# filippo-orru/path-tracer-rust

Hardware: AMD Instinct MI355X
Metric: ray_bounces_per_sec (higher is better)
Workload: dtype f32

## Files before the change

### path-tracer-rust_amd/csrc/pt_api.hip

```cpp
#include <cerrno>
#include <chrono>
#include <cstdio>
#include <cstdlib>
#include <cstring>
#include <map>
#include <string>
#include <thread>
#include <vector>

#include "../../include/ptrace.h"
#include "pt_accum.h"
#include "pt_aov.h"
#include "pt_denoise.h"
#include "pt_host.h"
#include "pt_kernels.h"
#include "pt_masked.h"
#include "pt_noise.h"
#include "pt_present.h"
#include "pt_probe.h"
#include "pt_refit.h"
#include "pt_reproject.h"
#include "pt_upsample.h"
#include "pt_tile.h"

// ... 1366 lines not shown
        HIP_TRY(hipMemcpy(c->d_sph.p, fs.sph_pairs.data(), fs.sph_pairs.size() * sizeof(SphPairRec), hipMemcpyHostToDevice));
    if (!fs.flat_pairs.empty())
        HIP_TRY(hipMemcpy(c->d_flat.p, fs.flat_pairs.data(), fs.flat_pairs.size() * sizeof(FlatPairRec), hipMemcpyHostToDevice));
    if (!fs.cand_pairs.empty())
        HIP_TRY(hipMemcpy(c->d_cand.p, fs.cand_pairs.data(), fs.cand_pairs.size() * sizeof(CandPairRec), hipMemcpyHostToDevice));
    HIP_TRY(hipMemcpy(c->d_rank_id.p, fs.rank_id.data(), fs.rank_id.size() * sizeof(uint32_t), hipMemcpyHostToDevice));
    c->scene.sph_pairs = c->d_sph.p;
    c->scene.flat_pairs = c->d_flat.p;
    c->scene.cand_pairs = c->d_cand.p;
    HIP_TRY(hipMemcpy(c->d_surf.p, fs.surf.data(), fs.surf.size() * sizeof(SurfRec), hipMemcpyHostToDevice));
    HIP_TRY(hipMemcpy(c->d_tri_rank.p, fs.tri_rank.data(), fs.tri_rank.size() * sizeof(uint32_t), hipMemcpyHostToDevice));
    c->scene.rank_id = c->d_rank_id.p;
    c->scene.tri_rank = c->d_tri_rank.p;
    if (!fs.bvh_meshes.empty())
        HIP_TRY(hipMemcpy(c->d_bvh_meshes.p, fs.bvh_meshes.data(), fs.bvh_meshes.size() * sizeof(BvhMeshRec), hipMemcpyHostToDevice));
    c->scene.bvh_meshes = c->d_bvh_meshes.p;
    c->scene.n_bvh_meshes = (uint32_t)fs.bvh_meshes.size();
    c->scene.surf = c->d_surf.p;
    c->scene.n_sph_pairs = (uint32_t)fs.sph_pairs.size();
    c->scene.n_flat_pairs = (uint32_t)fs.flat_pairs.size();
    c->scene.n_cand_pairs = (uint32_t)fs.cand_pairs.size();
    c->scene.n_other_pairs = fs.n_other_pairs;
    c->scene.n_flat_exact = fs.n_flat_exact;
    c->scene.nodes_in_lds_ok = c->tune.nodes_lds ? 1u : 0u;
    set_glass_defer(c, objs, n_objs);
    c->cand_ok = fs.cand_ok;
    c->scene.cand_staged = 0u;
    c->scene.surf_staged = 0u;
    c->scene.surf_head = 0u;
    c->scene.walk_queue_cap = c->tune.walk_queue_cap;
#ifdef PT_WALK_STATS
    if (!c->scene.stats) {
        HIP_TRY(hipMalloc((void **)&c->scene.stats, 16 * sizeof(unsigned long long)));
        HIP_TRY(hipMemset(c->scene.stats, 0, 16 * sizeof(unsigned long long)));
    }
#endif
#ifdef PT_PHASE_STATS
    if (!c->scene.phase_stats) {
        HIP_TRY(hipMalloc((void **)&c->scene.phase_stats, (kPhCount * 3 + 2) * sizeof(unsigned long long)));
        HIP_TRY(hipMemset(c->scene.phase_stats, 0, (kPhCount * 3 + 2) * sizeof(unsigned long long)));
    }
#endif
    c->n_bvh_nodes = (uint32_t)fs.bvh_nodes.size();
    c->scene.bvh_nodes = c->d_nodes.p;
    c->scene.n_bvh_nodes = c->n_bvh_nodes;
    c->scene.planar = 1u;
// ... 144 lines not shown
    if (moved) {
        HIP_TRY(hipMemcpy(c->d_opairs.p + e.obj_pair, &fs.obj_pairs[e.obj_pair], sizeof(ObjPairRec), hipMemcpyHostToDevice));
        if (e.on_device) {
            HIP_TRY(hipMemcpy(c->d_bvh_meshes.p + e.bvh_mesh, &fs.bvh_meshes[e.bvh_mesh], sizeof(BvhMeshRec), hipMemcpyHostToDevice));
        } else {
            int rc;
            if ((rc = c->d_sph.ensure(fs.sph_pairs.size())) || (rc = c->d_flat.ensure(fs.flat_pairs.size())) ||
                (rc = c->d_cand.ensure(fs.cand_pairs.size())))
                return rc;
            if (!fs.sph_pairs.empty())
                HIP_TRY(hipMemcpy(c->d_sph.p, fs.sph_pairs.data(), fs.sph_pairs.size() * sizeof(SphPairRec), hipMemcpyHostToDevice));
            if (!fs.flat_pairs.empty())
                HIP_TRY(hipMemcpy(c->d_flat.p, fs.flat_pairs.data(), fs.flat_pairs.size() * sizeof(FlatPairRec), hipMemcpyHostToDevice));
            if (!fs.cand_pairs.empty())
                HIP_TRY(hipMemcpy(c->d_cand.p, fs.cand_pairs.data(), fs.cand_pairs.size() * sizeof(CandPairRec), hipMemcpyHostToDevice));
            c->scene.sph_pairs = c->d_sph.p;
            c->scene.flat_pairs = c->d_flat.p;
            c->scene.cand_pairs = c->d_cand.p;
            c->scene.n_sph_pairs = (uint32_t)fs.sph_pairs.size();
            c->scene.n_flat_pairs = (uint32_t)fs.flat_pairs.size();
            c->scene.n_cand_pairs = (uint32_t)fs.cand_pairs.size();
            c->scene.n_other_pairs = fs.n_other_pairs;
            c->scene.n_flat_exact = fs.n_flat_exact;
            c->cand_ok = fs.cand_ok;
            c->scene.cand_scan = cand_scan_for(c, 0u);
            c->table_count[PT_TABLE_SPH_PAIRS] = fs.sph_pairs.size();
            c->table_count[PT_TABLE_FLAT_PAIRS] = fs.flat_pairs.size();
            c->table_count[PT_TABLE_CAND_PAIRS] = fs.cand_pairs.size();
            if (o.kind == PT_MESH && o.tri_count != 0u) {
                const ObjRec &r = fs.objs[index];
                HIP_TRY(hipMemcpy(c->d_tris.p + r.pair_begin, &fs.tri_pairs[r.pair_begin], (size_t)r.pair_count * sizeof(TriPairRec),
                                  hipMemcpyHostToDevice));
                HIP_TRY(hipMemcpy(c->d_tshade.p + o.tri_offset, &fs.tri_shade[o.tri_offset], (size_t)o.tri_count * sizeof(TriShade),
                                  hipMemcpyHostToDevice));
            }
        }
    }
    if (!e.surf.empty())
        HIP_TRY(hipMemcpy(c->d_surf.p + e.rank, e.surf.data(), e.surf.size() * sizeof(SurfRec), hipMemcpyHostToDevice));
    if (!e.tail.empty())
        HIP_TRY(hipMemcpy(c->d_surf.p + e.tail_at, e.tail.data(), e.tail.size() * sizeof(SurfRec), hipMemcpyHostToDevice));
    if (e.on_device) {
        if (moved) {
            pt_ctx::DevRefit *d = nullptr;
            const int rc = refit_plan_for(c, index, &d);
            if (rc) return rc;
// ... 1495 lines not shown
```

### path-tracer-rust_amd/csrc/pt_device.h

```cpp
#pragma once

#include "pt_math.h"

namespace pt {

constexpr uint32_t kKindSphere = 0u, kKindMesh = 1u;
constexpr uint32_t kDiffuse = 0u, kSpecular = 1u, kRefract = 2u;
constexpr int kMaxDepth = 12;

struct alignas(16) ObjRec {
    float cx, cy, cz;
    float rr;
    uint32_t kind;
    uint32_t tri_begin;
    uint32_t tri_count;
    uint32_t pair_begin;
    uint32_t pair_count;
    int32_t bvh_root;
    float rr_in;
    uint32_t pad1;
};

struct alignas(16) ObjPairRec {
    float cx[2], cy[2], cz[2];
    float rr[2];
// ... 106 lines not shown
    const TriShade *tri_shade;
    const BvhNode *bvh_nodes;
    const BvhNode4 *bvh_nodes4;
    uint32_t n_bvh_nodes4;
    uint32_t n_objs;
    uint32_t n_tris;
    uint32_t n_bvh_nodes;
    uint32_t bvh_in_lds;
    uint32_t bvh_pair_base;
    uint32_t bvh_stack;
    uint32_t leaf_quorum;
    uint32_t planar;
    const SphPairRec *sph_pairs;
    const FlatPairRec *flat_pairs;
    const CandPairRec *cand_pairs;
    const uint32_t *rank_id;
    const SurfRec *surf;
    const uint32_t *tri_rank;
    const BvhMeshRec *bvh_meshes;
    uint32_t n_bvh_meshes;
    uint32_t n_sph_pairs, n_flat_pairs, n_cand_pairs;
    uint32_t n_other_pairs;
    uint32_t n_flat_exact;
    uint32_t glass_defer_ok;
    uint32_t nodes_in_lds_ok;
    uint32_t cand_scan;
    uint32_t cand_staged;
    uint32_t surf_staged;
    uint32_t surf_head;
    uint32_t walk_queue_cap;
#ifdef PT_WALK_STATS
    unsigned long long *stats;
#endif
#ifdef PT_PHASE_STATS
    unsigned long long *phase_stats;
#endif
};
#ifdef PT_PHASE_STATS
enum : uint32_t {
    kPhOther = 0, kPhLoad, kPhSpheres, kPhFilter, kPhBatch, kPhFinish, kPhSurface, kPhRng, kPhDiffuse, kPhSpecular, kPhGlass,
    kPhAppend, kPhDefer, kPhBarrier, kPhWants, kPhWalkGate, kPhWalkBox, kPhWalkLeaf, kPhPrimary, kPhEmit,
    kPhPush, kPhAppend2, kPhRoulette, kPhEmitAdd, kPhCount
};
struct PhaseLds {
    unsigned long long state[4];
    unsigned long long cyc[4][kPhCount];
// ... 161 lines not shown
__device__ __forceinline__ void phase_end(unsigned long long *out, unsigned long long t0, unsigned long long r0) {
    phase_to(kPhOther);
    PhaseLds &P = phase_lds();
    const uint32_t w = threadIdx.x >> 6, lane = threadIdx.x & 63u;
    for (uint32_t k = lane; k < kPhCount; k += 64u) {
        const unsigned long long c = *(volatile unsigned long long *)&P.cyc[w][k], n = *(volatile unsigned long long *)&P.cnt[w][k];
        if (c) atomicAdd(out + 3u * k, c);
        if (n) {
            atomicAdd(out + 3u * k + 1u, n >> 32);
            atomicAdd(out + 3u * k + 2u, n & 0xffffffffull);
        }
    }
    if (lane == 0u) {
        atomicAdd(out + kPhCount * 3u, (unsigned long long)(__builtin_amdgcn_s_memtime() - t0));
        atomicAdd(out + kPhCount * 3u + 1u, (unsigned long long)(__builtin_amdgcn_s_memrealtime() - r0));
    }
}
#endif

typedef float f32x2 __attribute__((ext_vector_type(2)));
__device__ __forceinline__ f32x2 splat2(float v) {
    f32x2 r = {v, v};
    return r;
}
template <class T>
__device__ __forceinline__ T ld_uniform(const T *p) {
    static_assert(sizeof(T) % 16 == 0 && alignof(T) >= 16, "records are whole 16-byte rows");
    typedef uint32_t row_t __attribute__((ext_vector_type(4)));
    union {
        T v;
        row_t w[sizeof(T) / 16];
    } u;
    const __attribute__((address_space(4))) row_t *q =
        (const __attribute__((address_space(4))) row_t *)(unsigned long long)p;
#pragma unroll
    for (uint32_t i = 0; i < sizeof(T) / 16; ++i) u.w[i] = q[i];
    return u.v;
}
__device__ __forceinline__ f32x2 ld2(const float (&p)[2]) {
    f32x2 r = {p[0], p[1]};
    return r;
}
__device__ __forceinline__ f32x2 f_rcp2(f32x2 d) {
    const f32x2 one = splat2(1.0f);
    const f32x2 r0 = {__builtin_amdgcn_rcpf(d[0]), __builtin_amdgcn_rcpf(d[1])};
    const f32x2 e0 = __builtin_elementwise_fma(-d, r0, one);
// ... 818 lines not shown
            const float sq = f_sqrt(det);
            suspect = !(!(det < 0.0f) && ((b - sq) >= 1e-4f || (b + sq) >= 1e-4f));
        }
    }
    if (__builtin_amdgcn_ballot_w64(suspect) != 0ull) h = scan_scene<BVH, true, DEFER_WALK>(S, o, d, lds, want_walk);
    return h;
}

struct CandLds {
    unsigned long long *keys;
    float4 *ray_a;
    float2 *ray_b;
    uint16_t *queue;
    const CandPairRec *staged;
    const SurfRec *surf;
};
constexpr unsigned long long kKeyMiss = 0x7f800000ffffffffull;

struct CandRing {
    uint32_t head, count;
};

template <int AXIS, bool EXACT>
__device__ __forceinline__ void filter_flat(const FlatPairRec &f, vec3 o, vec3 d, vec3 inv, float bound, uint64_t valid_m,
                                            uint64_t graze, uint64_t *m0, uint64_t *m1) {
    const float oa = AXIS == 0 ? o.x : (AXIS == 1 ? o.y : o.z), ob = AXIS == 0 ? o.y : (AXIS == 1 ? o.z : o.x),
                oc = AXIS == 0 ? o.z : (AXIS == 1 ? o.x : o.y);
    const float db = AXIS == 0 ? d.y : (AXIS == 1 ? d.z : d.x), dc = AXIS == 0 ? d.z : (AXIS == 1 ? d.x : d.y);
    const float ia = AXIS == 0 ? inv.x : (AXIS == 1 ? inv.y : inv.z);
    const f32x2 tv = ld2(f.pc) - splat2(oa);
    const f32x2 t2 = tv * splat2(ia);
    const f32x2 yb = __builtin_elementwise_fma(splat2(db), t2, splat2(ob)) - ld2(f.cb);
    const f32x2 zc = __builtin_elementwise_fma(splat2(dc), t2, splat2(oc)) - ld2(f.cc);
    const f32x2 lim = splat2(bound) + ld2(f.tpad);
    uint64_t in[2];
    if (EXACT) {
#pragma unroll
        for (int hf = 0; hf < 2; ++hf)
            in[hf] = __builtin_amdgcn_ballot_w64(f_abs(yb[hf]) <= f.hb[hf]) & __builtin_amdgcn_ballot_w64(f_abs(zc[hf]) <= f.hc[hf]) &
                     __builtin_amdgcn_ballot_w64(t2[hf] <= lim[hf]);
        const uint64_t fwd0 = __builtin_amdgcn_ballot_w64(t2[0] > 0.0f), fwd1 = __builtin_amdgcn_ballot_w64(t2[1] > 0.0f);
        *m0 = f.pair[0] != kNoPair ? ((graze | in[0]) & fwd0 & valid_m) : 0ull;
        *m1 = f.pair[1] != kNoPair ? ((graze | in[1]) & fwd1 & valid_m) : 0ull;
        return;
    }
#pragma unroll
    for (int hf = 0; hf < 2; ++hf)
        in[hf] = __builtin_amdgcn_ballot_w64(f_abs(yb[hf]) <= f.hb[hf]) & __builtin_amdgcn_ballot_w64(f_abs(zc[hf]) <= f.hc[hf]) &
                 __builtin_amdgcn_ballot_w64(t2[hf] >= -f.tpad[hf]) & __builtin_amdgcn_ballot_w64(t2[hf] <= lim[hf]);
    *m0 = f.pair[0] != kNoPair ? ((graze | in[0]) & valid_m) : 0ull;
    *m1 = f.pair[1] != kNoPair ? ((graze | in[1]) & valid_m) : 0ull;
}

__device__ __forceinline__ unsigned long long cand_spheres(const DevScene &S, vec3 o, vec3 d, float *best_out) {
    float best_t = __builtin_inff();
    uint32_t best_rank = 0xffffffffu;
    const f32x2 ox2 = splat2(o.x), oy2 = splat2(o.y), oz2 = splat2(o.z);
    const f32x2 dx2 = splat2(d.x), dy2 = splat2(d.y), dz2 = splat2(d.z);
    for (uint32_t p = 0; p < S.n_sph_pairs; ++p) {
        const SphPairRec sp = ld_uniform(S.sph_pairs + p);
        const f32x2 opx = ld2(sp.cx) - ox2, opy = ld2(sp.cy) - oy2, opz = ld2(sp.cz) - oz2;
        const f32x2 b = (opx * dx2 + opy * dy2) + opz * dz2;
        const f32x2 det = (b * b - ((opx * opx + opy * opy) + opz * opz)) + ld2(sp.rr);
#pragma unroll
        for (int hf = 0; hf < 2; ++hf) {
            if (__builtin_amdgcn_ballot_w64(!(det[hf] < 0.0f)) == 0ull) continue;
            const float sq = f_sqrt(det[hf]);
            const float t0 = b[hf] - sq, t1 = b[hf] + sq;
            const bool near_ok = t0 >= 1e-4f, far_ok = t1 >= 1e-4f;
            const float t = near_ok ? t0 : t1;
            if (far_ok && t < best_t) {
                best_t = t;
                best_rank = sp.rank[hf];
            }
        }
    }
    *best_out = best_t;
    return ((unsigned long long)__float_as_uint(best_t) << 32) | best_rank;
}

template <bool STAGED>
__device__ __forceinline__ void cand_batch(const DevScene &S, const CandLds &L, CandRing &R, uint32_t lane, uint32_t count) {
    PT_PHASE_N(kPhBatch, count);
    const bool valid = lane < count;
    const uint32_t at = (R.head + lane) & (kCandQueueCap - 1u);
    R.head = (R.head + count) & (kCandQueueCap - 1u);
    R.count -= count;
    if (valid) {
        const uint32_t ent = (uint32_t)L.queue[at];
        const uint32_t slot = ent & 127u, q = ent >> 7;
        const float4 ra = L.ray_a[slot];
        const float2 rb = L.ray_b[slot];
        const vec3 ro = mk(ra.x, ra.y, ra.z), rd = mk(ra.w, rb.x, rb.y);
        CandPairRec tr;
        if (STAGED)
            tr = L.staged[q];
        else
            tr = S.cand_pairs[q];
        unsigned long long keys2[2];
        float t_hit[2];
        pair_test_keys(tr, ro, rd, keys2, t_hit);
        const bool first = keys2[0] <= keys2[1];
        const unsigned long long kmin = first ? keys2[0] : keys2[1];
        const float mt = first ? t_hit[0] : t_hit[1];
        bool pass = (uint32_t)(kmin >> 32) < 0x7f800000u;
        const vec3 g = mk(tr.gx, tr.gy, tr.gz);
        const vec3 pc = (ro + rd * mt) - g;
        const bool deep = dot(pc, pc) <= tr.grr_in;
        if (pass && !deep) {
            const vec3 og = g - ro;
            const float b = dot(og, rd);
            const float det = (b * b - dot(og, og)) + tr.grr;
            const float sq = f_sqrt(det);
            pass = !(det < 0.0f) && ((b - sq) >= 1e-4f || (b + sq) >= 1e-4f);
        }
        if (pass) atomicMin(&L.keys[slot], kmin + (1ull << 32));
    }
}

template <bool STAGED>
__device__ __forceinline__ void cand_filter_and_drain(const DevScene &S, const CandLds &L, CandRing &R, uint32_t lane,
                                                      uint32_t par, bool valid, vec3 o, vec3 d, float bound) {
    auto push2 = [&](uint64_t m0, uint32_t q0, uint64_t m1, uint32_t q1) {
        if ((m0 | m1) == 0ull) return;
        const uint32_t n0 = (uint32_t)__builtin_popcountll(m0);
        const uint32_t base = R.head + R.count;
        const uint32_t me = lane | (par << 6);
        if (__builtin_amdgcn_inverse_ballot_w64(m0)) {
            PT_PHASE(kPhPush);
            const uint32_t at = (base + __builtin_amdgcn_mbcnt_hi((uint32_t)(m0 >> 32), __builtin_amdgcn_mbcnt_lo((uint32_t)m0, 0u))) & (kCandQueueCap - 1u);
            L.queue[at] = (uint16_t)(me | (q0 << 7));
        }
        if (__builtin_amdgcn_inverse_ballot_w64(m1)) {
            PT_PHASE(kPhPush);
            const uint32_t at = (base + n0 + __builtin_amdgcn_mbcnt_hi((uint32_t)(m1 >> 32), __builtin_amdgcn_mbcnt_lo((uint32_t)m1, 0u))) & (kCandQueueCap - 1u);
            L.queue[at] = (uint16_t)(me | (q1 << 7));
        }
        PT_PHASE(kPhFilter);
        R.count += n0 + (uint32_t)__builtin_popcountll(m1);
    };
    auto drain = [&]() {
#ifdef PT_PHASE_STATS
        const bool any = R.count >= 64u;
#endif
        while (R.count >= 64u) cand_batch<STAGED>(S, L, R, lane, 64u);
#ifdef PT_PHASE_STATS
        if (any) PT_PHASE(kPhFilter);
#endif
    };
    PT_PHASE(kPhFilter);
    const vec3 inv = mk(__builtin_amdgcn_rcpf(d.x), __builtin_amdgcn_rcpf(d.y), __builtin_amdgcn_rcpf(d.z));
    const uint64_t valid_m = __builtin_amdgcn_ballot_w64(valid);
    const uint64_t gz_x = __builtin_amdgcn_ballot_w64(!(f_abs(d.x) >= kGrazing)), gz_y = __builtin_amdgcn_ballot_w64(!(f_abs(d.y) >= kGrazing)),
                   gz_z = __builtin_amdgcn_ballot_w64(!(f_abs(d.z) >= kGrazing));
    for (uint32_t p = 0; p < S.n_flat_exact; ++p) {
        const FlatPairRec f = ld_uniform(S.flat_pairs + p);
        uint64_t m0, m1;
        if (f.axis == 0u)
            filter_flat<0, true>(f, o, d, inv, bound, valid_m, gz_x, &m0, &m1);
        else if (f.axis == 1u)
            filter_flat<1, true>(f, o, d, inv, bound, valid_m, gz_y, &m0, &m1);
        else
            filter_flat<2, true>(f, o, d, inv, bound, valid_m, gz_z, &m0, &m1);
        push2(m0, f.pair[0], m1, f.pair[1]);
        drain();
    }
    for (uint32_t p = S.n_flat_exact; p < S.n_flat_pairs; ++p) {
        const FlatPairRec f = ld_uniform(S.flat_pairs + p);
        uint64_t m0, m1;
        if (f.axis == 0u)
            filter_flat<0, false>(f, o, d, inv, bound, valid_m, gz_x, &m0, &m1);
        else if (f.axis == 1u)
            filter_flat<1, false>(f, o, d, inv, bound, valid_m, gz_y, &m0, &m1);
        else
            filter_flat<2, false>(f, o, d, inv, bound, valid_m, gz_z, &m0, &m1);
        push2(m0, f.pair[0], m1, f.pair[1]);
        drain();
    }
    for (uint32_t q = 0; q < S.n_other_pairs; ++q) {
        push2(valid_m, q, 0ull, 0u);
        drain();
    }
}

__device__ __forceinline__ bool walk_deferred(const DevScene &S, vec3 o, vec3 d, uint4 *lds, float &best_t,
                                              int32_t &best_id, const LeafLds *leaves = nullptr) {
    bool tie = false;
    const uint32_t n_pairs = (S.n_objs + 1u) >> 1;
    for (uint32_t p = 0; p < n_pairs; ++p) {
        const ObjPairRec ob = ld_uniform(S.obj_pairs + p);
#pragma unroll
        for (int hf = 0; hf < 2; ++hf) {
            const int32_t root = ob.bvh_root[hf];
            if (ob.kind[hf] != kKindMesh || root == kNoBvh) continue;
            const vec3 op = mk(ob.cx[hf], ob.cy[hf], ob.cz[hf]) - o;
            const float b = dot(op, d);
            const float det = (b * b - dot(op, op)) + ob.rr[hf];
            const float sq = f_sqrt(det);
            const bool pass = !(det < 0.0f) && ((b - sq) >= 1e-4f || (b + sq) >= 1e-4f);
            if (__builtin_amdgcn_ballot_w64(pass) == 0ull) continue;
            float mt = __builtin_inff();
            int32_t mid = -1;
            if (pass) {
                bvh_walk(S, lds, o, d, root, best_t, mt, mid, leaves);
            }
// ... 317 lines not shown
```

### path-tracer-rust_amd/csrc/pt_host.cpp

```cpp
#include "pt_host.h"
#include "pt_denoise.h"
#include "pt_masked.h"
#include "pt_present.h"
#include "pt_probe.h"
#include "pt_refit.h"
#include "pt_reproject.h"
#include "pt_upsample.h"

#include <algorithm>
#include <cmath>
#include <cstring>
#include <limits>

namespace pt {
namespace host {

static vec3 ld(const float *p) { return mk(p[0], p[1], p[2]); }
static void st(float *p, vec3 v) {
    p[0] = v.x;
    p[1] = v.y;
    p[2] = v.z;
}

void camera_basis(const pt_camera &cam, float lens_center[3], float su_out[3], float sv_out[3]) {
// ... 486 lines not shown
                const uint32_t hf = fill[a] & 1u;
                f.pc[hf] = lov[a];
                f.cb[hf] = 0.5f * (lov[b] + hiv[b]);
                f.hb[hf] = 0.5f * (hiv[b] - lov[b]) + pad + 4.0f * e * (f_abs(lov[b]) + f_abs(hiv[b]));
                f.cc[hf] = 0.5f * (lov[c] + hiv[c]);
                f.hc[hf] = 0.5f * (hiv[c] - lov[c]) + pad + 4.0f * e * (f_abs(lov[c]) + f_abs(hiv[c]));
                f.tpad[hf] = pad;
                for (int h2 = 0; h2 < 2; ++h2) {
                    if (tp.id[h2] == kNoTri) continue;
                    const float e1v[3] = {tp.e1x[h2], tp.e1y[h2], tp.e1z[h2]}, e2v[3] = {tp.e2x[h2], tp.e2y[h2], tp.e2z[h2]};
                    const double pa = (double)e1v[b] * e2v[c], pb = (double)e1v[c] * e2v[b];
                    if (!(std::fabs(pa - pb) >= 1e-3 * (std::fabs(pa) + std::fabs(pb))) || !std::isfinite(pa) || !std::isfinite(pb))
                        f.sign_exact = 0u;
                }
                f.pair[hf] = (uint32_t)filtered.size();
                filtered.push_back(cand_rec(i, pp));
                ++fill[a];
            }
        }
        for (int a = 0; a < 3; ++a) out.flat_pairs.insert(out.flat_pairs.end(), by_axis[a].begin(), by_axis[a].end());
        out.n_flat_exact = (uint32_t)(std::stable_partition(out.flat_pairs.begin(), out.flat_pairs.end(),
                                                            [](const FlatPairRec &f) { return f.sign_exact != 0u; }) -
                                      out.flat_pairs.begin());
        out.n_other_pairs = (uint32_t)out.cand_pairs.size();
        for (FlatPairRec &f : out.flat_pairs)
            for (int hf = 0; hf < 2; ++hf)
                if (f.pair[hf] != kNoPair) f.pair[hf] += out.n_other_pairs;
        out.cand_pairs.insert(out.cand_pairs.end(), filtered.begin(), filtered.end());
        out.cand_ok = out.cand_pairs.size() <= kCandMaxPairs;
    }
}

const char *bad_material(const pt_object &o) {
    for (float v : o.color)
        if (!finite_nonneg(v)) return "color";
    for (float v : o.emission)
        if (!finite_nonneg(v)) return "emission";
    return nullptr;
}

bool flatten_scene(const pt_camera &cam, const pt_object *objs, uint32_t n_objs, const pt_triangle *tris,
                   uint32_t n_tris, FlatScene &out, std::string &err, const Reach *origin_box, Reach *used) {
    if (n_objs >= (1u << 30) || n_tris >= (1u << 30)) {
        err = "scene too large";
        return false;
    }
// ... 1129 lines not shown
```

### path-tracer-rust_amd/csrc/pt_host.h

```cpp
#pragma once

#include <algorithm>
#include <string>
#include <vector>

#include "../../include/ptrace.h"
#include "pt_device.h"
#include "pt_refit.h"

namespace pt {

void set_error(const std::string &m);
inline int refuse(const char *why) {
    set_error(why);
    return PT_ERR_INVALID;
}

namespace host {

struct FlatScene {
    std::vector<ObjRec> objs;
    std::vector<ObjPairRec> obj_pairs;
    std::vector<TriPairRec> tri_pairs;
    std::vector<MatRec> mats;
    std::vector<TriShade> tri_shade;
    std::vector<BvhNode> bvh_nodes;
    std::vector<BvhNode4> bvh_nodes4;
    std::vector<SphPairRec> sph_pairs;
    std::vector<FlatPairRec> flat_pairs;
    std::vector<CandPairRec> cand_pairs;
    std::vector<uint32_t> rank_id;
    std::vector<SurfRec> surf;
    std::vector<uint32_t> tri_rank;
    std::vector<BvhMeshRec> bvh_meshes;
    std::vector<uint32_t> wide_src;
    uint32_t n_other_pairs = 0;
    uint32_t n_flat_exact = 0;
    bool cand_ok = false;
    uint32_t bvh_stack = 0;
    uint32_t bvh_pair_base = 0;
    uint32_t bvh_pair_span = 0;
};

void camera_basis(const pt_camera &cam, float lens_center[3], float su[3], float sv[3]);
void mesh_bounding_sphere(const pt_triangle *tris, uint32_t n, float center[3], float *radius);
void mesh_bounding_box(const pt_triangle *tris, uint32_t n, pt_triangle out[12]);
void box_pair_records(const pt_triangle box[12], const float position[3], TriPairRec out[6]);
bool bvh_refs_fit(uint64_t n_nodes, uint64_t n_pair_records);

struct PassPlanIn {
    uint64_t npix = 0;
    uint32_t spp = 0;
    uint64_t want = 0;
    bool want_is_default = true;
    bool stack_form = false;
    bool stack_park = false;
    bool cand_scan = false, has_bvh = false;
    uint64_t streams = 0;
    uint32_t per_stream = 0;
    uint32_t wave_stack = 0;
// ... 211 lines not shown
```

### path-tracer-rust_amd/csrc/pt_kernels.hip

```cpp
#include <cstdio>
#include <cstdlib>
#include <string>

#include "pt_kernels.h"
#ifdef PT_TU_TILE
#include "pt_tile.h"
#endif

namespace pt {

#ifdef PT_TU_TILE
typedef TileParams MegaParams;
#define k_mega k_tile_mega
#define k_mega_cand k_tile_mega_cand
#else
typedef FrameParams MegaParams;
#endif
#if defined(PT_TU_FLAT) || defined(PT_TU_TILE)
#define PT_TU_PART 1
#endif

void set_error(const std::string &m);

extern __shared__ uint4 dyn_lds[];
// ... 12 lines not shown
__device__ __forceinline__ StreamSlice slice_of(const RayQueue &q, uint32_t b, uint32_t cap) {
    StreamSlice s;
    s.base = q.buf + (size_t)b * cap * kRayBytes;
    s.off_tp = cap * 16u;
    s.off_od1 = cap * 32u;
    return s;
}
__device__ __forceinline__ float4 ld_od0(const StreamSlice &q, uint32_t i) { return *reinterpret_cast<const float4 *>(q.base + i * 16u); }
__device__ __forceinline__ float4 ld_tp(const StreamSlice &q, uint32_t i) { return *reinterpret_cast<const float4 *>(q.base + (i * 16u + q.off_tp)); }
__device__ __forceinline__ float2 ld_od1(const StreamSlice &q, uint32_t i) { return *reinterpret_cast<const float2 *>(q.base + (i * 8u + q.off_od1)); }
__device__ __forceinline__ void store_ray(const StreamSlice &q, uint32_t slot, vec3 o, vec3 d, vec3 thr, uint32_t word) {
    *reinterpret_cast<float4 *>(q.base + slot * 16u) = make_float4(o.x, o.y, o.z, d.x);
    *reinterpret_cast<float2 *>(q.base + (slot * 8u + q.off_od1)) = make_float2(d.y, d.z);
    *reinterpret_cast<float4 *>(q.base + (slot * 16u + q.off_tp)) = make_float4(thr.x, thr.y, thr.z, __uint_as_float(word));
}
__device__ __forceinline__ void load_ray_slice(const StreamSlice &q, uint32_t i, vec3 &o, vec3 &d, vec3 &thr, uint32_t &word) {
    const float4 a = ld_od0(q, i);
    const float4 tp = ld_tp(q, i);
    const float2 c = ld_od1(q, i);
    o = mk(a.x, a.y, a.z);
    d = mk(a.w, c.x, c.y);
    thr = mk(tp.x, tp.y, tp.z);
    word = __float_as_uint(tp.w);
}

#ifndef PT_TU_PART
template <bool PROBE>
__global__ __launch_bounds__(kBlock) void k_generate(FrameParams F, RayQueue q, uint32_t *__restrict__ cnt0,
                                                     uint32_t cap, uint32_t s0, uint32_t s_here, uint32_t m) {
    const uint32_t b = blockIdx.x, tid = threadIdx.x;
    const StreamSlice qs = slice_of(q, b, cap);
    const uint32_t mb = stream_pixel_count(F.npix, F.n_streams, b);
    const uint32_t n = mb * s_here;
    for (uint32_t g = tid; g < n; g += kBlock) {
        const uint32_t pl = stream_pixel(F.n_streams, b, g % mb);
        const uint32_t s = s0 + g / mb;
        const PathRay r = primary_ray<PROBE>(F, global_pixel(F, pl), s);
        store_ray(qs, g, r.o, r.d, r.thr, pack_word(g % mb, g / mb, PROBE ? F.depth0 : 0u, 1u));
    }
    if (tid == 0) cnt0[b] = n;
}

constexpr uint32_t kParkCap = 128;
__host__ __device__ inline size_t bvh_park_offset(const DevScene &S, uint32_t block) {
    return (bvh_lds_bytes(S, block) + 15) & ~(size_t)15;
}
// ... 657 lines not shown
        const uint32_t phi = 2u * top + 4u * (n_park + n_defer + (pending ? 64u : 0u));
        const bool may_start = gen_left != 0u && (room_for_all || phi + 256u <= room);
        uint32_t src = 0u, cnt = 0u;
        if (top >= 64u) {
            src = 1u;
            cnt = 64u;
        } else if (may_start) {
            src = 2u;
            cnt = gen_left < 64u ? gen_left : 64u;
        } else if (top != 0u) {
            src = 1u;
            cnt = top;
        }
        src = rfl(src);
        cnt = rfl(cnt);
        const bool idle = src == 0u && !pending;
        if (idle && n_defer == 0u && n_park == 0u) break;
        const bool cur_valid = lane < cnt;
        vec3 cur_thr = mk(0.0f, 0.0f, 0.0f);
        uint32_t word = 0;
        const uint32_t pend_entries = ring.count;
        bool ran_batch = false;
        if (src != 0u) {
            PathRay in;
            in.o = in.d = in.thr = mk(0.0f, 0.0f, 0.0f);
            if (src == 2u) {
                PT_PHASE(kPhPrimary);
                if (cur_valid) {
                    const uint32_t pj = gen_pj, sj = gen_sj;
                    FrameParams Fl;
                    {
                        const float4 c0 = *reinterpret_cast<const float4 *>(s_tail_p + 4), c1 = *reinterpret_cast<const float4 *>(s_tail_p + 8),
                                     c2 = *reinterpret_cast<const float4 *>(s_tail_p + 12);
                        Fl.lens_x = c0.x, Fl.lens_y = c0.y, Fl.lens_z = c0.z, Fl.cam_px = c0.w, Fl.cam_py = c1.x, Fl.cam_pz = c1.y;
                        Fl.su_x = c1.z, Fl.su_y = c1.w, Fl.su_z = c2.x, Fl.sv_x = c2.y, Fl.sv_y = c2.z, Fl.sv_z = c2.w;
                        Fl.width = s_tail_p[16], Fl.height = s_tail_p[17];
                        Fl.seed_lo = P.seed_lo, Fl.seed_hi = P.seed_hi;
                    }
                    in = PROBE ? primary_ray<PROBE>(F, lds_pix[pj], s0 + sj) : primary_ray_at(Fl, lds_pix[pj], lds_px[pj], lds_py[pj], s0 + sj);
                    word = pack_word(pj, sj, PROBE ? F.depth0 : 0u, 1u);
                }
#if PT_SAMPLE_MAJOR
                gen_sj += step_r;
                gen_pj += step_q;
                if (gen_sj >= s_here) {
                    gen_sj -= s_here;
                    gen_pj += 1u;
                }
#else
                gen_pj += step_r;
                gen_sj += step_q;
                if (gen_pj >= mb) {
                    gen_pj -= mb;
                    gen_sj += 1u;
                }
#endif
                gen_left = rfl(gen_left - cnt);
            } else {
                PT_PHASE(kPhLoad);
                __builtin_amdgcn_fence(__ATOMIC_RELEASE, "wavefront");
                __builtin_amdgcn_fence(__ATOMIC_ACQUIRE, "wavefront");
                top = rfl(top - cnt);
                if (cur_valid) load_ray_slice(qs, top + lane, in.o, in.d, in.thr, word);
            }
            total += cnt;
            cur_thr = in.thr;
            const uint32_t slot = (par << 6) | lane;
            cand.ray_a[slot] = make_float4(in.o.x, in.o.y, in.o.z, in.d.x);
            cand.ray_b[slot] = make_float2(in.d.y, in.d.z);
            float bound;
            PT_PHASE(kPhSpheres);
            const unsigned long long key0 = cand_spheres(S, in.o, in.d, &bound);
            cand.keys[slot] = cur_valid ? key0 : kKeyMiss;
            const uint32_t before = ring.head;
            cand_filter_and_drain<STAGED>(S, cand, ring, lane, par, cur_valid, in.o, in.d, bound);
            ran_batch = ring.head != before;
        }
        if (pending) {
            PT_PHASE(kPhFinish);
            if (pend_entries != 0u && !ran_batch) cand_batch<STAGED>(S, cand, ring, lane, ring.count);
            PT_PHASE(kPhFinish);
            ShadeOut so;
            so.n_rays = 0;
            so.emits = false;
            so.deferred = false;
            float hit_t = 0.0f;
            uint32_t hit_rank = 0xffffffffu;
            PathRay pr;
            pr.o = pr.d = pr.thr = mk(0.0f, 0.0f, 0.0f);
            bool park = false;
            unsigned long long park_key = 0ull;
            if (prev_valid) {
                const uint32_t slot = ((par ^ 1u) << 6) | lane;
                const unsigned long long key = load_key(&cand.keys[slot]);
                const uint32_t rank = (uint32_t)key;
                if (BVH) {
                    const float4 ra = cand.ray_a[slot];
                    const float2 rb = cand.ray_b[slot];
// ... 1146 lines not shown
```

### path-tracer-rust_amd/host/object_check.cpp

```cpp
#include "check_common.h"
#include "../csrc/pt_host.h"

using namespace pt;
using host::FlatScene;
using host::Reach;

template <class T>
static bool same_table(const std::vector<T> &a, const std::vector<T> &b) {
    return a.size() == b.size() && (a.empty() || memcmp(a.data(), b.data(), a.size() * sizeof(T)) == 0);
}

struct Scene {
    pt_camera cam;
    std::vector<pt_object> objs;
    std::vector<pt_triangle> tris;
};

static void terrain(uint32_t q, uint32_t n, uint32_t seed, std::vector<pt_triangle> &out) {
    std::vector<float> h((size_t)(q + 1u) * (q + 1u));
    uint32_t s = seed;
    for (float &v : h) v = (float)(lcg(s) >> 26) * 0.125f;
    auto vert = [&](uint32_t i, uint32_t j, float v[3]) {
        v[0] = (float)i * 0.375f - 1.0f, v[1] = h[(size_t)i * (q + 1u) + j], v[2] = (float)j * 0.625f - 2.0f;
    };
// ... 55 lines not shown
static bool flatten(const Scene &sc, FlatScene &fs, const Reach *B, Reach *used) {
    std::string err;
    return host::flatten_scene(sc.cam, sc.objs.data(), (uint32_t)sc.objs.size(), sc.tris.data(), (uint32_t)sc.tris.size(), fs, err, B, used);
}

static bool same_tables(const FlatScene &a, const FlatScene &b) {
    const struct {
        const char *name;
        bool same;
    } t[] = {{"objs", same_table(a.objs, b.objs)},
             {"obj_pairs", same_table(a.obj_pairs, b.obj_pairs)},
             {"tri_pairs", same_table(a.tri_pairs, b.tri_pairs)},
             {"mats", same_table(a.mats, b.mats)},
             {"tri_shade", same_table(a.tri_shade, b.tri_shade)},
             {"bvh_nodes", same_table(a.bvh_nodes, b.bvh_nodes)},
             {"bvh_nodes4", same_table(a.bvh_nodes4, b.bvh_nodes4)},
             {"sph_pairs", same_table(a.sph_pairs, b.sph_pairs)},
             {"flat_pairs", same_table(a.flat_pairs, b.flat_pairs)},
             {"cand_pairs", same_table(a.cand_pairs, b.cand_pairs)},
             {"rank_id", same_table(a.rank_id, b.rank_id)},
             {"surf", same_table(a.surf, b.surf)},
             {"tri_rank", same_table(a.tri_rank, b.tri_rank)},
             {"bvh_meshes", same_table(a.bvh_meshes, b.bvh_meshes)},
             {"the counts", a.n_other_pairs == b.n_other_pairs && a.n_flat_exact == b.n_flat_exact && a.cand_ok == b.cand_ok}};
    for (const auto &x : t)
        if (!x.same) {
            fprintf(stderr, "same_tables: %s differ\n", x.name);
            return false;
        }
    return true;
}

static bool same_small_tables(const FlatScene &a, const FlatScene &b) {
    return same_table(a.mats, b.mats) && same_table(a.tri_shade, b.tri_shade) && same_table(a.sph_pairs, b.sph_pairs) &&
           same_table(a.flat_pairs, b.flat_pairs) && same_table(a.cand_pairs, b.cand_pairs) && same_table(a.surf, b.surf) &&
           a.n_other_pairs == b.n_other_pairs && a.n_flat_exact == b.n_flat_exact && a.cand_ok == b.cand_ok;
}

static bool same_spheres(const FlatScene &a, const FlatScene &b) {
    if (a.objs.size() != b.objs.size() || a.bvh_meshes.size() != b.bvh_meshes.size()) return false;
    for (size_t i = 0; i < a.objs.size(); ++i) {
        const float x[5] = {a.objs[i].cx, a.objs[i].cy, a.objs[i].cz, a.objs[i].rr, a.objs[i].rr_in};
        const float y[5] = {b.objs[i].cx, b.objs[i].cy, b.objs[i].cz, b.objs[i].rr, b.objs[i].rr_in};
        const ObjPairRec &p = a.obj_pairs[(a.objs.size() - 1u - i) / 2u], &q = b.obj_pairs[(a.objs.size() - 1u - i) / 2u];
        const size_t hf = (a.objs.size() - 1u - i) & 1u;
        if (memcmp(x, y, sizeof x) != 0 || p.cx[hf] != q.cx[hf] || p.cy[hf] != q.cy[hf] || p.cz[hf] != q.cz[hf] || p.rr[hf] != q.rr[hf] ||
            p.admit[hf] != q.admit[hf] || p.obj[hf] != q.obj[hf])
            return false;
    }
    for (size_t m = 0; m < a.bvh_meshes.size(); ++m)
        if (memcmp(&a.bvh_meshes[m], &b.bvh_meshes[m], 4 * sizeof(float)) != 0) return false;
    return true;
}

static bool refit_is_sound(const FlatScene &a, const FlatScene &b, const Scene &sc, const Reach &B) {
    const float scene_R = length(mk(B.hi[0] - B.lo[0], B.hi[1] - B.lo[1], B.hi[2] - B.lo[2]));
    std::vector<const TriPairRec *> rec_b(sc.tris.size(), nullptr);
    std::vector<uint32_t> half_b(sc.tris.size(), 0u), owner(sc.tris.size(), 0u);
    for (const TriPairRec &r : b.tri_pairs)
// ... 266 lines not shown
```

Before: 56.00 billion.

## Pack ray into paired registers and split exact flat filtering per axis

Ray origin and direction are carried as three packed float pairs, with empty asm pins so the compiler keeps them as paired VGPRs for packed math in the sphere and flat-pair filter loops. The exact flat-pair loop is split into three axis-specialised runs using per-axis counts computed on the host, which removes the per-pair axis branch. The ray slice load becomes unconditional with a clamped lane index, and the valid mask comes from a lane-count compare instead of a ballot. The per-axis loops assume exact pairs are grouped by axis after the host partition. Pinning may also raise register pressure.

```diff
diff --git a/path-tracer-rust_amd/csrc/pt_api.hip b/path-tracer-rust_amd/csrc/pt_api.hip
--- a/path-tracer-rust_amd/csrc/pt_api.hip
+++ b/path-tracer-rust_amd/csrc/pt_api.hip
@@ -1412,6 +1412,7 @@
     c->scene.n_cand_pairs = (uint32_t)fs.cand_pairs.size();
     c->scene.n_other_pairs = fs.n_other_pairs;
     c->scene.n_flat_exact = fs.n_flat_exact;
+    for (int k = 0; k < 3; ++k) c->scene.n_flat_exact_axis[k] = fs.n_flat_exact_axis[k];
     c->scene.nodes_in_lds_ok = c->tune.nodes_lds ? 1u : 0u;
     set_glass_defer(c, objs, n_objs);
     c->cand_ok = fs.cand_ok;
@@ -1602,6 +1603,7 @@
             c->scene.n_cand_pairs = (uint32_t)fs.cand_pairs.size();
             c->scene.n_other_pairs = fs.n_other_pairs;
             c->scene.n_flat_exact = fs.n_flat_exact;
+            for (int k = 0; k < 3; ++k) c->scene.n_flat_exact_axis[k] = fs.n_flat_exact_axis[k];
             c->cand_ok = fs.cand_ok;
             c->scene.cand_scan = cand_scan_for(c, 0u);
             c->table_count[PT_TABLE_SPH_PAIRS] = fs.sph_pairs.size();
diff --git a/path-tracer-rust_amd/csrc/pt_device.h b/path-tracer-rust_amd/csrc/pt_device.h
--- a/path-tracer-rust_amd/csrc/pt_device.h
+++ b/path-tracer-rust_amd/csrc/pt_device.h
@@ -1,6 +1,8 @@
 #pragma once
 
 #include "pt_math.h"
+
+#include <type_traits>
 
 namespace pt {
 
@@ -153,6 +155,7 @@
     uint32_t n_sph_pairs, n_flat_pairs, n_cand_pairs;
     uint32_t n_other_pairs;
     uint32_t n_flat_exact;
+    uint32_t n_flat_exact_axis[3];
     uint32_t glass_defer_ok;
     uint32_t nodes_in_lds_ok;
     uint32_t cand_scan;
@@ -360,6 +363,49 @@
 __device__ __forceinline__ f32x2 splat2(float v) {
     f32x2 r = {v, v};
     return r;
+}
+typedef float f32x4 __attribute__((ext_vector_type(4)));
+struct RayRows {
+    f32x2 p0, p1;
+    f32x2 p2;
+};
+enum : int { kRayOx = 0, kRayOy, kRayOz, kRayDx, kRayDy, kRayDz };
+__device__ __forceinline__ RayRows ray_rows(vec3 o, vec3 d) {
+    RayRows r;
+    r.p0 = f32x2{o.x, o.y};
+    r.p1 = f32x2{o.z, d.x};
+    r.p2 = f32x2{d.y, d.z};
+    return r;
+}
+template <int C>
+__device__ __forceinline__ float ray_get(const RayRows &r) {
+    static_assert(C >= 0 && C < 6, "o.x, o.y, o.z, d.x, d.y, d.z");
+    if constexpr (C < 2)
+        return r.p0[C];
+    else if constexpr (C < 4)
+        return r.p1[C - 2];
+    else
+        return r.p2[C - 4];
+}
+__device__ __forceinline__ void pin_pair(f32x2 &p) { asm volatile("" : "+v"(p)); }
+__device__ __forceinline__ void pin_rows(RayRows &r) {
+    pin_pair(r.p0);
+    pin_pair(r.p1);
+    pin_pair(r.p2);
+}
+template <int H>
+__device__ __forceinline__ f32x2 rep2(f32x2 p) {
+    return __builtin_shufflevector(p, p, H, H);
+}
+template <int C>
+__device__ __forceinline__ f32x2 ray_rep(const RayRows &r) {
+    static_assert(C >= 0 && C < 6, "o.x, o.y, o.z, d.x, d.y, d.z");
+    if constexpr (C < 2)
+        return rep2<C>(r.p0);
+    else if constexpr (C < 4)
+        return rep2<C - 2>(r.p1);
+    else
+        return rep2<C - 4>(r.p2);
 }
 template <class T>
 __device__ __forceinline__ T ld_uniform(const T *p) {
@@ -1224,17 +1270,21 @@
 };
 
 template <int AXIS, bool EXACT>
-__device__ __forceinline__ void filter_flat(const FlatPairRec &f, vec3 o, vec3 d, vec3 inv, float bound, uint64_t valid_m,
+__device__ __forceinline__ void filter_flat(const FlatPairRec &f, const RayRows &ray, f32x2 inv_xy, f32x2 inv_zb, uint64_t valid_m,
                                             uint64_t graze, uint64_t *m0, uint64_t *m1) {
-    const float oa = AXIS == 0 ? o.x : (AXIS == 1 ? o.y : o.z), ob = AXIS == 0 ? o.y : (AXIS == 1 ? o.z : o.x),
-                oc = AXIS == 0 ? o.z : (AXIS == 1 ? o.x : o.y);
-    const float db = AXIS == 0 ? d.y : (AXIS == 1 ? d.z : d.x), dc = AXIS == 0 ? d.z : (AXIS == 1 ? d.x : d.y);
-    const float ia = AXIS == 0 ? inv.x : (AXIS == 1 ? inv.y : inv.z);
-    const f32x2 tv = ld2(f.pc) - splat2(oa);
-    const f32x2 t2 = tv * splat2(ia);
-    const f32x2 yb = __builtin_elementwise_fma(splat2(db), t2, splat2(ob)) - ld2(f.cb);
-    const f32x2 zc = __builtin_elementwise_fma(splat2(dc), t2, splat2(oc)) - ld2(f.cc);
-    const f32x2 lim = splat2(bound) + ld2(f.tpad);
+    constexpr int A = AXIS, B = (AXIS + 1) % 3, C = (AXIS + 2) % 3;
+    const f32x2 oa = ray_rep<kRayOx + A>(ray), ob = ray_rep<kRayOx + B>(ray), oc = ray_rep<kRayOx + C>(ray);
+    const f32x2 db = ray_rep<kRayDx + B>(ray), dc = ray_rep<kRayDx + C>(ray);
+    f32x2 ia;
+    if constexpr (A < 2)
+        ia = rep2<A>(inv_xy);
+    else
+        ia = rep2<0>(inv_zb);
+    const f32x2 tv = ld2(f.pc) - oa;
+    const f32x2 t2 = tv * ia;
+    const f32x2 yb = __builtin_elementwise_fma(db, t2, ob) - ld2(f.cb);
+    const f32x2 zc = __builtin_elementwise_fma(dc, t2, oc) - ld2(f.cc);
+    const f32x2 lim = rep2<1>(inv_zb) + ld2(f.tpad);
     uint64_t in[2];
     if (EXACT) {
 #pragma unroll
@@ -1254,13 +1304,14 @@
     *m1 = f.pair[1] != kNoPair ? ((graze | in[1]) & valid_m) : 0ull;
 }
 
-__device__ __forceinline__ unsigned long long cand_spheres(const DevScene &S, vec3 o, vec3 d, float *best_out) {
+__device__ __forceinline__ unsigned long long cand_spheres(const DevScene &S, RayRows &r, float *best_out) {
     float best_t = __builtin_inff();
     uint32_t best_rank = 0xffffffffu;
-    const f32x2 ox2 = splat2(o.x), oy2 = splat2(o.y), oz2 = splat2(o.z);
-    const f32x2 dx2 = splat2(d.x), dy2 = splat2(d.y), dz2 = splat2(d.z);
     for (uint32_t p = 0; p < S.n_sph_pairs; ++p) {
         const SphPairRec sp = ld_uniform(S.sph_pairs + p);
+        pin_rows(r);
+        const f32x2 ox2 = ray_rep<kRayOx>(r), oy2 = ray_rep<kRayOy>(r), oz2 = ray_rep<kRayOz>(r);
+        const f32x2 dx2 = ray_rep<kRayDx>(r), dy2 = ray_rep<kRayDy>(r), dz2 = ray_rep<kRayDz>(r);
         const f32x2 opx = ld2(sp.cx) - ox2, opy = ld2(sp.cy) - oy2, opz = ld2(sp.cz) - oz2;
         const f32x2 b = (opx * dx2 + opy * dy2) + opz * dz2;
         const f32x2 det = (b * b - ((opx * opx + opy * opy) + opz * opz)) + ld2(sp.rr);
@@ -1279,6 +1330,10 @@
     }
     *best_out = best_t;
     return ((unsigned long long)__float_as_uint(best_t) << 32) | best_rank;
+}
+__device__ __forceinline__ unsigned long long cand_spheres(const DevScene &S, vec3 o, vec3 d, float *best_out) {
+    RayRows r = ray_rows(o, d);
+    return cand_spheres(S, r, best_out);
 }
 
 template <bool STAGED>
@@ -1322,7 +1377,7 @@
 
 template <bool STAGED>
 __device__ __forceinline__ void cand_filter_and_drain(const DevScene &S, const CandLds &L, CandRing &R, uint32_t lane,
-                                                      uint32_t par, bool valid, vec3 o, vec3 d, float bound) {
+                                                      uint32_t par, uint64_t valid_m, const RayRows &ray, float bound) {
     auto push2 = [&](uint64_t m0, uint32_t q0, uint64_t m1, uint32_t q1) {
         if ((m0 | m1) == 0ull) return;
         const uint32_t n0 = (uint32_t)__builtin_popcountll(m0);
@@ -1351,31 +1406,36 @@
 #endif
     };
     PT_PHASE(kPhFilter);
-    const vec3 inv = mk(__builtin_amdgcn_rcpf(d.x), __builtin_amdgcn_rcpf(d.y), __builtin_amdgcn_rcpf(d.z));
-    const uint64_t valid_m = __builtin_amdgcn_ballot_w64(valid);
-    const uint64_t gz_x = __builtin_amdgcn_ballot_w64(!(f_abs(d.x) >= kGrazing)), gz_y = __builtin_amdgcn_ballot_w64(!(f_abs(d.y) >= kGrazing)),
-                   gz_z = __builtin_amdgcn_ballot_w64(!(f_abs(d.z) >= kGrazing));
-    for (uint32_t p = 0; p < S.n_flat_exact; ++p) {
+    const float dx = ray_get<kRayDx>(ray), dy = ray_get<kRayDy>(ray), dz = ray_get<kRayDz>(ray);
+    f32x2 inv_xy = {__builtin_amdgcn_rcpf(dx), __builtin_amdgcn_rcpf(dy)};
+    f32x2 inv_zb = {__builtin_amdgcn_rcpf(dz), bound};
+    RayRows r = ray;
+    const uint64_t gz_x = __builtin_amdgcn_ballot_w64(!(f_abs(dx) >= kGrazing)), gz_y = __builtin_amdgcn_ballot_w64(!(f_abs(dy) >= kGrazing)),
+                   gz_z = __builtin_amdgcn_ballot_w64(!(f_abs(dz) >= kGrazing));
+    uint32_t p = 0;
+    auto run_axis = [&](auto axis, uint32_t n, uint64_t graze) {
+        for (const uint32_t end = p + n; p < end; ++p) {
+            const FlatPairRec f = ld_uniform(S.flat_pairs + p);
+            pin_rows(r), pin_pair(inv_xy), pin_pair(inv_zb);
+            uint64_t m0, m1;
+            filter_flat<decltype(axis)::value, true>(f, r, inv_xy, inv_zb, valid_m, graze, &m0, &m1);
+            push2(m0, f.pair[0], m1, f.pair[1]);
+            drain();
+        }
+    };
+    run_axis(std::integral_constant<int, 0>(), S.n_flat_exact_axis[0], gz_x);
+    run_axis(std::integral_constant<int, 1>(), S.n_flat_exact_axis[1], gz_y);
+    run_axis(std::integral_constant<int, 2>(), S.n_flat_exact_axis[2], gz_z);
+    for (; p < S.n_flat_pairs; ++p) {
         const FlatPairRec f = ld_uniform(S.flat_pairs + p);
+        pin_rows(r), pin_pair(inv_xy), pin_pair(inv_zb);
         uint64_t m0, m1;
         if (f.axis == 0u)
-            filter_flat<0, true>(f, o, d, inv, bound, valid_m, gz_x, &m0, &m1);
+            filter_flat<0, false>(f, r, inv_xy, inv_zb, valid_m, gz_x, &m0, &m1);
         else if (f.axis == 1u)
-            filter_flat<1, true>(f, o, d, inv, bound, valid_m, gz_y, &m0, &m1);
+            filter_flat<1, false>(f, r, inv_xy, inv_zb, valid_m, gz_y, &m0, &m1);
         else
-            filter_flat<2, true>(f, o, d, inv, bound, valid_m, gz_z, &m0, &m1);
-        push2(m0, f.pair[0], m1, f.pair[1]);
-        drain();
-    }
-    for (uint32_t p = S.n_flat_exact; p < S.n_flat_pairs; ++p) {
-        const FlatPairRec f = ld_uniform(S.flat_pairs + p);
-        uint64_t m0, m1;
-        if (f.axis == 0u)
-            filter_flat<0, false>(f, o, d, inv, bound, valid_m, gz_x, &m0, &m1);
-        else if (f.axis == 1u)
-            filter_flat<1, false>(f, o, d, inv, bound, valid_m, gz_y, &m0, &m1);
-        else
-            filter_flat<2, false>(f, o, d, inv, bound, valid_m, gz_z, &m0, &m1);
+            filter_flat<2, false>(f, r, inv_xy, inv_zb, valid_m, gz_z, &m0, &m1);
         push2(m0, f.pair[0], m1, f.pair[1]);
         drain();
     }
@@ -1383,6 +1443,11 @@
         push2(valid_m, q, 0ull, 0u);
         drain();
     }
+}
+template <bool STAGED>
+__device__ __forceinline__ void cand_filter_and_drain(const DevScene &S, const CandLds &L, CandRing &R, uint32_t lane,
+                                                      uint32_t par, bool valid, vec3 o, vec3 d, float bound) {
+    cand_filter_and_drain<STAGED>(S, L, R, lane, par, (uint64_t)__builtin_amdgcn_ballot_w64(valid), ray_rows(o, d), bound);
 }
 
 __device__ __forceinline__ bool walk_deferred(const DevScene &S, vec3 o, vec3 d, uint4 *lds, float &best_t,
diff --git a/path-tracer-rust_amd/csrc/pt_host.cpp b/path-tracer-rust_amd/csrc/pt_host.cpp
--- a/path-tracer-rust_amd/csrc/pt_host.cpp
+++ b/path-tracer-rust_amd/csrc/pt_host.cpp
@@ -532,6 +532,8 @@
         out.n_flat_exact = (uint32_t)(std::stable_partition(out.flat_pairs.begin(), out.flat_pairs.end(),
                                                             [](const FlatPairRec &f) { return f.sign_exact != 0u; }) -
                                       out.flat_pairs.begin());
+        for (uint32_t &n : out.n_flat_exact_axis) n = 0u;
+        for (uint32_t k = 0; k < out.n_flat_exact; ++k) ++out.n_flat_exact_axis[out.flat_pairs[k].axis];
         out.n_other_pairs = (uint32_t)out.cand_pairs.size();
         for (FlatPairRec &f : out.flat_pairs)
             for (int hf = 0; hf < 2; ++hf)
diff --git a/path-tracer-rust_amd/csrc/pt_host.h b/path-tracer-rust_amd/csrc/pt_host.h
--- a/path-tracer-rust_amd/csrc/pt_host.h
+++ b/path-tracer-rust_amd/csrc/pt_host.h
@@ -36,6 +36,7 @@
     std::vector<uint32_t> wide_src;
     uint32_t n_other_pairs = 0;
     uint32_t n_flat_exact = 0;
+    uint32_t n_flat_exact_axis[3] = {0, 0, 0};
     bool cand_ok = false;
     uint32_t bvh_stack = 0;
     uint32_t bvh_pair_base = 0;
diff --git a/path-tracer-rust_amd/csrc/pt_kernels.hip b/path-tracer-rust_amd/csrc/pt_kernels.hip
--- a/path-tracer-rust_amd/csrc/pt_kernels.hip
+++ b/path-tracer-rust_amd/csrc/pt_kernels.hip
@@ -58,6 +58,13 @@
     d = mk(a.w, c.x, c.y);
     thr = mk(tp.x, tp.y, tp.z);
     word = __float_as_uint(tp.w);
+}
+__device__ __forceinline__ void load_ray_slice(const StreamSlice &q, uint32_t i, RayRows &ray, f32x4 &tp) {
+    const f32x2 *a = reinterpret_cast<const f32x2 *>(q.base + i * 16u);
+    ray.p0 = a[0];
+    ray.p1 = a[1];
+    tp = *reinterpret_cast<const f32x4 *>(q.base + (i * 16u + q.off_tp));
+    ray.p2 = *reinterpret_cast<const f32x2 *>(q.base + (i * 8u + q.off_od1));
 }
 
 #ifndef PT_TU_PART
@@ -761,10 +768,11 @@
         const uint32_t pend_entries = ring.count;
         bool ran_batch = false;
         if (src != 0u) {
-            PathRay in;
-            in.o = in.d = in.thr = mk(0.0f, 0.0f, 0.0f);
+            RayRows ray;
             if (src == 2u) {
                 PT_PHASE(kPhPrimary);
+                PathRay in;
+                in.o = in.d = in.thr = mk(0.0f, 0.0f, 0.0f);
                 if (cur_valid) {
                     const uint32_t pj = gen_pj, sj = gen_sj;
                     FrameParams Fl;
@@ -795,24 +803,28 @@
                 }
 #endif
                 gen_left = rfl(gen_left - cnt);
+                ray = ray_rows(in.o, in.d);
+                cur_thr = in.thr;
             } else {
                 PT_PHASE(kPhLoad);
                 __builtin_amdgcn_fence(__ATOMIC_RELEASE, "wavefront");
                 __builtin_amdgcn_fence(__ATOMIC_ACQUIRE, "wavefront");
                 top = rfl(top - cnt);
-                if (cur_valid) load_ray_slice(qs, top + lane, in.o, in.d, in.thr, word);
+                f32x4 tp;
+                load_ray_slice(qs, top + (lane < cnt - 1u ? lane : cnt - 1u), ray, tp);
+                cur_thr = mk(tp[0], tp[1], tp[2]);
+                word = __float_as_uint(tp[3]);
             }
             total += cnt;
-            cur_thr = in.thr;
             const uint32_t slot = (par << 6) | lane;
-            cand.ray_a[slot] = make_float4(in.o.x, in.o.y, in.o.z, in.d.x);
-            cand.ray_b[slot] = make_float2(in.d.y, in.d.z);
+            cand.ray_a[slot] = make_float4(ray.p0[0], ray.p0[1], ray.p1[0], ray.p1[1]);
+            cand.ray_b[slot] = make_float2(ray.p2[0], ray.p2[1]);
             float bound;
             PT_PHASE(kPhSpheres);
-            const unsigned long long key0 = cand_spheres(S, in.o, in.d, &bound);
+            const unsigned long long key0 = cand_spheres(S, ray, &bound);
             cand.keys[slot] = cur_valid ? key0 : kKeyMiss;
             const uint32_t before = ring.head;
-            cand_filter_and_drain<STAGED>(S, cand, ring, lane, par, cur_valid, in.o, in.d, bound);
+            cand_filter_and_drain<STAGED>(S, cand, ring, lane, par, __builtin_amdgcn_uicmp(lane, cnt, 36 ), ray, bound);
             ran_batch = ring.head != before;
         }
         if (pending) {
diff --git a/path-tracer-rust_amd/host/object_check.cpp b/path-tracer-rust_amd/host/object_check.cpp
--- a/path-tracer-rust_amd/host/object_check.cpp
+++ b/path-tracer-rust_amd/host/object_check.cpp
@@ -1,3 +1,5 @@
+#include <algorithm>
+
 #include "check_common.h"
 #include "../csrc/pt_host.h"
 
@@ -101,7 +103,8 @@
              {"surf", same_table(a.surf, b.surf)},
              {"tri_rank", same_table(a.tri_rank, b.tri_rank)},
              {"bvh_meshes", same_table(a.bvh_meshes, b.bvh_meshes)},
-             {"the counts", a.n_other_pairs == b.n_other_pairs && a.n_flat_exact == b.n_flat_exact && a.cand_ok == b.cand_ok}};
+             {"the counts", a.n_other_pairs == b.n_other_pairs && a.n_flat_exact == b.n_flat_exact &&
+                  std::equal(a.n_flat_exact_axis, a.n_flat_exact_axis + 3, b.n_flat_exact_axis) && a.cand_ok == b.cand_ok}};
     for (const auto &x : t)
         if (!x.same) {
             fprintf(stderr, "same_tables: %s differ\n", x.name);
@@ -113,7 +116,8 @@
 static bool same_small_tables(const FlatScene &a, const FlatScene &b) {
     return same_table(a.mats, b.mats) && same_table(a.tri_shade, b.tri_shade) && same_table(a.sph_pairs, b.sph_pairs) &&
            same_table(a.flat_pairs, b.flat_pairs) && same_table(a.cand_pairs, b.cand_pairs) && same_table(a.surf, b.surf) &&
-           a.n_other_pairs == b.n_other_pairs && a.n_flat_exact == b.n_flat_exact && a.cand_ok == b.cand_ok;
+           a.n_other_pairs == b.n_other_pairs && a.n_flat_exact == b.n_flat_exact &&
+           std::equal(a.n_flat_exact_axis, a.n_flat_exact_axis + 3, b.n_flat_exact_axis) && a.cand_ok == b.cand_ok;
 }
 
 static bool same_spheres(const FlatScene &a, const FlatScene &b) {
```

Result: faster. 58.66 billion (median of 6 runs) (+4.8%).
